# vmonardo/pnp-svrg

Hardware: AMD Instinct MI355X
Metric: PnP-SVRG inner-iters/sec, 256x256 CSMRI+DnCNN (higher is better)
Workload: dtype f32; 1 GPU; pnp_svrg (true SVRG direction, T2=10, mb=1000) on 256x256 CSMRI, 20% Bernoulli mask, DnCNN-17 prox (reference DnCNN_noise15 weights); batch_per_gpu=120, problems_total=120, parallelism=replicas x1 (no data-path collective)

## Files before the change

### pnp_svrg_amd/csrc/dncnn_wino44.hip

```cpp
#include "common.h"
#include "wino44.h"
#include "tilewalk.h"
#include <vector>
#include <utility>
#include <cstdlib>

namespace pnp {
namespace w44 {

using f32x4 = __attribute__((ext_vector_type(4))) float;
using f32x2 = __attribute__((ext_vector_type(2))) float;

constexpr int C = 64;
constexpr int TC = 64;
constexpr int PC = 72;
constexpr int KC = 8;
constexpr int NCH = C / KC;
template <int NG_> struct Geo {
    static constexpr int NG = NG_;
    static constexpr int TR = 4 * NG, PR = TR + 2;
    static constexpr int PLANE = NG == 2 ? 768 : 512;
    static constexpr int DBUF = KC * PLANE;
    static constexpr int PPW = DBUF / 256 / 4;
    static constexpr int VPL = 128 * NG;
    static constexpr int VBUF = 36 * VPL;
    static constexpr int LDS_FLOATS = 2 * DBUF + 2 * VBUF;
    static constexpr int NQ_AGPR = NG == 2 ? 64 : 36;
    static constexpr bool in_agpr(int g, int xi) { return g * 36 + xi < NQ_AGPR; }
};
constexpr int URING = 18;
constexpr unsigned DUMMY = 1u << 27;

__device__ __forceinline__ void bt6(float d0, float d1, float d2, float d3, float d4, float d5, float (&v)[6]) {
    const float t1 = __builtin_fmaf(-4.f, d2, d4), t2 = __builtin_fmaf(-4.f, d1, d3);
    const float t3 = d4 - d2, sd = d3 - d1;
    v[0] = __builtin_fmaf(4.f, d0, __builtin_fmaf(-5.f, d2, d4));
    v[1] = t1 + t2;
    v[2] = t1 - t2;
    v[3] = __builtin_fmaf(2.f, sd, t3);
    v[4] = __builtin_fmaf(-2.f, sd, t3);
    v[5] = __builtin_fmaf(4.f, d1, __builtin_fmaf(-5.f, d3, d5));
}
template <typename T> __device__ __forceinline__ void at6(T m0, T m1, T m2, T m3, T m4, T m5, T (&y)[4]) {
    const T s12 = m1 + m2, d12 = m1 - m2, s34 = m3 + m4, d34 = m3 - m4;
    y[0] = (m0 + s12) + s34;
    y[1] = 2.f * d34 + d12;
    y[2] = 4.f * s34 + s12;
    y[3] = (8.f * d34 + d12) + m5;
}

#define PNP_MFMA_PRE ""
#define PNP_MFMA_POST ""
template <bool AG> __device__ __forceinline__ void mfma(f32x4& acc, float w, float v) {
    if (AG) asm volatile(PNP_MFMA_PRE "v_mfma_f32_16x16x4_f32 %0, %1, %2, %0" PNP_MFMA_POST : "+a"(acc) : "v"(w), "v"(v));
    else asm volatile(PNP_MFMA_PRE "v_mfma_f32_16x16x4_f32 %0, %1, %2, %0" PNP_MFMA_POST : "+v"(acc) : "v"(w), "v"(v));
}
template <bool AG> __device__ __forceinline__ void mfma_first(f32x4& acc, float w, float v) {
    if (AG) asm volatile("v_mfma_f32_16x16x4_f32 %0, %1, %2, 0" PNP_MFMA_POST : "=&a"(acc) : "v"(w), "v"(v));
    else asm volatile("v_mfma_f32_16x16x4_f32 %0, %1, %2, 0" PNP_MFMA_POST : "=&v"(acc) : "v"(w), "v"(v));
}

typedef int i32x4 __attribute__((ext_vector_type(4)));
typedef __attribute__((address_space(3))) float lds_f;
typedef __attribute__((address_space(3))) f32x2 lds_f2;
typedef __attribute__((address_space(3))) f32x4 lds_f4;

__device__ __forceinline__ void dma_piece_asm(unsigned voff, i32x4 rsrc, unsigned lds_byte_addr) {
    asm volatile("s_mov_b32 m0, %2\n\ts_nop 0\n\tbuffer_load_dwordx4 %0, %1, 0 offen lds" :: "v"(voff), "s"(rsrc), "s"(lds_byte_addr) : "memory");
}

struct Patch {
    f32x2 a; f32x4 m; f32x2 e;
    f32x2 t[6][3];
    f32x2 v[6];
};
template <int NG_> struct Ctx {
    static constexpr int NG = NG_;
    using G = Geo<NG_>;
    f32x4 acc[NG_][36];
    f32x4 ur[URING];
    Patch P;
    f32x2 b[2][NG_];
    const lds_f* dsrc[2];
    lds_f* vdst[2];
    const lds_f* vsrc0[2];
    const lds_f* vsrc1[2];
    const __attribute__((address_space(1))) char* ucur;
    unsigned ulane;
    __device__ __forceinline__ f32x4 uload_next() {
        const f32x4 u = *(const __attribute__((address_space(1))) f32x4*)(ucur + ulane);
        ucur += 1024;
        asm volatile("" : "+s"(ucur));
        return u;
    }
};
#define PNP_SLOT() __builtin_amdgcn_sched_barrier(0)

template <int DPAR, int R, int HALF, typename CT> __device__ __forceinline__ void patch_load(CT& c) {
    const lds_f* row = c.dsrc[DPAR] + R * PC;
    if (HALF == 0) { c.P.a = *(const lds_f2*)(row + 2); c.P.e = *(const lds_f2*)(row + 8); }
    else c.P.m = *(const lds_f4*)(row + 4);
}
__device__ __forceinline__ f32x2 pk_sum_diff(f32x2 a) {
    f32x2 r;
    asm("v_pk_add_f32 %0, %1, %1 op_sel:[0,1] op_sel_hi:[1,0] neg_hi:[0,1]" : "=v"(r) : "v"(a));
    return r;
}
__device__ __forceinline__ f32x2 pk_hi_pm_2lo(f32x2 a) {
    f32x2 r;
    asm("v_pk_fma_f32 %0, %1, 2.0, %1 op_sel:[0,0,1] op_sel_hi:[0,0,1] neg_hi:[1,0,0]" : "=v"(r) : "v"(a));
    return r;
}
__device__ __forceinline__ void bt6_pk(f32x2 q0, f32x2 q1, f32x2 q2, f32x2 q3, f32x2 q4, f32x2 q5, f32x2 (&v)[6]) {
    const f32x2 t1 = q4 - 4.f * q2, t2 = q3 - 4.f * q1;
    const f32x2 t3 = q4 - q2, sd = q3 - q1;
    v[0] = 4.f * q0 + (q4 - 5.f * q2);
    v[1] = t1 + t2;
    v[2] = t1 - t2;
    v[3] = 2.f * sd + t3;
    v[4] = t3 - 2.f * sd;
    v[5] = 4.f * q1 + (q5 - 5.f * q3);
}
constexpr int col_pair(int sl) { return (sl - 6) / 2; }
constexpr bool is_col_slice(int sl) { return sl == 6 || sl == 8 || sl == 10; }
template <int SL, typename CT> __device__ __forceinline__ void slice_valu(CT& c) {
    Patch& P = c.P;
    if constexpr (SL < 6) {
        asm volatile("" :: "v"(P.a.x), "v"(P.e.y));
        const f32x2 p12 = {P.m.x, P.m.y}, p34 = {P.m.z, P.m.w};
        const f32x2 A = p34 - 4.f * p12;
        const f32x2 Bv = p34 - p12;
        P.t[SL][1] = pk_sum_diff(A);
        P.t[SL][2] = pk_hi_pm_2lo(Bv);
        float v0, v5;
        asm("v_fma_f32 %0, 4.0, %1, %2" : "=v"(v0) : "v"(P.a.y), "v"(__builtin_fmaf(-5.f, P.m.y, P.m.w)));
        asm("v_fma_f32 %0, 4.0, %1, %2" : "=v"(v5) : "v"(P.m.x), "v"(__builtin_fmaf(-5.f, P.m.z, P.e.x)));
        P.t[SL][0] = f32x2{v0, v5};
    } else if constexpr (is_col_slice(SL)) {
        constexpr int cp = col_pair(SL);
        bt6_pk(P.t[0][cp], P.t[1][cp], P.t[2][cp], P.t[3][cp], P.t[4][cp], P.t[5][cp], P.v);
    }
}
template <int DPAR, int SL, int N, typename CT> __device__ __forceinline__ void slice_lds(CT& c) {
    constexpr int VPL = CT::G::VPL;
    if constexpr (SL < 5) {
        if constexpr (N < 2) patch_load<DPAR, SL + 1, N>(c);
    } else if constexpr (is_col_slice(SL)) {
        constexpr int cp = col_pair(SL), xa = cp == 0 ? 0 : cp == 1 ? 1 : 3, xb = cp == 0 ? 5 : cp == 1 ? 2 : 4;
#pragma unroll
        for (int y = 2 * N; y < 2 * N + 2; ++y) {
            c.vdst[DPAR][(y * 6 + xa) * VPL] = c.P.v[y].x;
            c.vdst[DPAR][(y * 6 + xb) * VPL] = c.P.v[y].y;
        }
    }
}
template <int VPAR, int XI, int GR, typename CT> __device__ __forceinline__ void b_load(CT& c) {
    if constexpr (GR < CT::NG) {
        if (GR == 0) c.b[XI & 1][0] = *(const lds_f2*)(c.vsrc0[VPAR] + XI * CT::G::VPL);
        else c.b[XI & 1][GR] = *(const lds_f2*)(c.vsrc1[VPAR] + XI * CT::G::VPL);
    }
}
template <int K, int XI, int GR, typename CT> __device__ __forceinline__ void mfma_j0(CT& c, float u, f32x2 (&b)[CT::NG]) {
    if constexpr (GR < CT::NG) {
        if constexpr (K == 0) mfma_first<CT::G::in_agpr(GR, XI)>(c.acc[GR][XI], u, b[GR].x);
        else mfma<CT::G::in_agpr(GR, XI)>(c.acc[GR][XI], u, b[GR].x);
    }
}
template <int XI, int GR, typename CT> __device__ __forceinline__ void mfma_j1(CT& c, float u, f32x2 (&b)[CT::NG]) {
    if constexpr (GR < CT::NG) mfma<CT::G::in_agpr(GR, XI)>(c.acc[GR][XI], u, b[GR].y);
}

template <int K, int P, int VAR, typename CT, typename DMA> __device__ __forceinline__ void step(CT& c, DMA&& dma) {
    constexpr int X0 = 2 * P, X1 = 2 * P + 1, SQ = K * 18 + P;
    constexpr int VPAR = K & 1, DPAR = (K + 1) & 1, NG = CT::NG;
    const f32x4 u = c.ur[SQ % URING];
    f32x2 b0[NG], b1[NG];
#pragma unroll
    for (int g = 0; g < NG; ++g) b0[g] = c.b[0][g];
    mfma_j0<K, X0, 0>(c, u.x, b0);                   PNP_SLOT();
    if constexpr (VAR != 13 && VAR != 15) b_load<VPAR, X1, 0>(c);
    PNP_SLOT();
    mfma_j0<K, X0, 1>(c, u.x, b0);                   PNP_SLOT();
    if constexpr (VAR != 13 && VAR != 15) b_load<VPAR, X1, 1>(c);
    PNP_SLOT();
    mfma_j1<X0, 0>(c, u.y, b0);                      PNP_SLOT();
    if constexpr (VAR != 10 && VAR != 15) slice_valu<P>(c);
    PNP_SLOT();
    mfma_j1<X0, 1>(c, u.y, b0);                      PNP_SLOT();
    if constexpr (VAR != 14 && VAR != 15) slice_lds<DPAR, P, 0>(c);
    PNP_SLOT();
#pragma unroll
    for (int g = 0; g < NG; ++g) b1[g] = c.b[1][g];
    mfma_j0<K, X1, 0>(c, u.z, b1);                   PNP_SLOT();
    if constexpr (X1 + 1 < 36 && VAR != 13 && VAR != 15) b_load<VPAR, X1 + 1, 0>(c);
    PNP_SLOT();
    mfma_j0<K, X1, 1>(c, u.z, b1);                   PNP_SLOT();
    if constexpr (X1 + 1 < 36 && VAR != 13 && VAR != 15) b_load<VPAR, X1 + 1, 1>(c);
    PNP_SLOT();
    mfma_j1<X1, 0>(c, u.w, b1);                      PNP_SLOT();
    if constexpr (P < CT::G::PPW && VAR != 11 && VAR != 15) dma(P);
    if constexpr (VAR != 14 && VAR != 15) slice_lds<DPAR, P, 1>(c);
    PNP_SLOT();
    mfma_j1<X1, 1>(c, u.w, b1);                      PNP_SLOT();
    if constexpr (VAR != 14 && VAR != 15) slice_lds<DPAR, P, 2>(c);
    if constexpr (VAR != 12 && VAR != 15 && SQ + URING < NCH * 18) c.ur[SQ % URING] = c.uload_next();
    PNP_SLOT();
}
template <int K, int VAR, typename CT, typename DMA, int... P> __device__ __forceinline__ void chunk_steps(CT& c, DMA&& dma, std::integer_sequence<int, P...>) {
    (step<K, P, VAR>(c, dma), ...);
}
template <int K> constexpr int reloads_from(int p0) {
    int n = 0;
    for (int p = p0; p < 18; ++p) n += (K * 18 + p + URING < NCH * 18) ? 1 : 0;
    return n;
}
template <int K, bool STAMP, int VAR, typename CT, typename DMA> __device__ __forceinline__ void chunk(CT& c, DMA&& dma, unsigned long long& t_wait) {
    patch_load<(K + 1) & 1, 0, 0>(c);
    patch_load<(K + 1) & 1, 0, 1>(c);
    b_load<K & 1, 0, 0>(c);
    b_load<K & 1, 0, 1>(c);
    PNP_SLOT();
    chunk_steps<K, VAR>(c, dma, std::make_integer_sequence<int, 18>{});
    unsigned long long ta = 0;
    if (STAMP) ta = __builtin_amdgcn_s_memtime();
    asm volatile("s_waitcnt vmcnt(%0)" :: "n"(reloads_from<K>(CT::G::PPW)) : "memory");
    __syncthreads();
    if (STAMP) t_wait += __builtin_amdgcn_s_memtime() - ta;
}
template <bool STAMP, int VAR, typename CT, typename MK, int... K> __device__ __forceinline__ void all_chunks(CT& c, MK&& mk, unsigned long long& t_wait, std::integer_sequence<int, K...>) {
    (chunk<K, STAMP, VAR>(c, mk(std::integral_constant<int, K>{}), t_wait), ...);
}

template <int VPL> __device__ __forceinline__ void transform0(const float* dsrc, float* vdst) {
    float t[6][6];
#pragma unroll
    for (int r = 0; r < 6; ++r) {
        const float* row = dsrc + r * PC;
        bt6(row[3], row[4], row[5], row[6], row[7], row[8], t[r]);
    }
#pragma unroll
    for (int x = 0; x < 6; ++x) {
        float v[6];
        bt6(t[0][x], t[1][x], t[2][x], t[3][x], t[4][x], t[5][x], v);
#pragma unroll
        for (int y = 0; y < 6; ++y) vdst[(y * 6 + x) * VPL] = v[y];
    }
}

constexpr int FL_PATCH = 36;
constexpr int FL_BLK = 16 * FL_PATCH;
template <int NG, bool FL> constexpr int fl_lds_floats() { return FL ? C * 9 + NG * 4 * FL_BLK : 0; }

template <bool LEAKY, int NG = 2, bool STAMP = false, int VAR = 0, bool FL = false>
__global__ __launch_bounds__(256, 1) void k_mid_wino44(const float* __restrict__ in, float* __restrict__ out,
                                                       const float4* __restrict__ upack, const float* __restrict__ bias,
                                                       int H, int W, int ntiles, float slope,
                                                       unsigned long long* __restrict__ stamps = nullptr, int tile0 = 0,
                                                       const float* __restrict__ wlast = nullptr, float* __restrict__ part = nullptr) {
    using G = Geo<NG>;
    constexpr int TR = G::TR, PR = G::PR, PLANE = G::PLANE, DBUF = G::DBUF, PPW = G::PPW, VPL = G::VPL, VBUF = G::VBUF;
    static_assert(!(FL && LEAKY), "the fused last layer is built for the ReLU net");
    __shared__ __attribute__((aligned(16))) float lds[G::LDS_FLOATS + fl_lds_floats<NG, FL>()];
    const int tid = threadIdx.x, lane = tid & 63, wv = __builtin_amdgcn_readfirstlane(tid >> 6);
    const int tiles_x = W / TC, units_per_img = tiles_x * (H / 8);
    auto region = [&](int u, int& b, int& ty0, int& tx0) {
        const int t = tile0 + (NG == 2 ? u : u >> 1);
        b = t / units_per_img;
        const int t2 = t - b * units_per_img;
        ty0 = (t2 / tiles_x) * 8 + (NG == 2 ? 0 : 4 * (u & 1));
        tx0 = (t2 % tiles_x) * TC;
    };

    float bv[4];
#pragma unroll
    for (int r = 0; r < 4; ++r) bv[r] = bias[16 * wv + 4 * (lane >> 4) + r];

    const int tc = lane & 15, j = (lane >> 4) & 1, g = NG == 2 ? lane >> 5 : 0;
    const int d_off = 4 * ((2 * wv + j) * (PLANE / 4) + g * PC + tc);
    const ptrdiff_t hw4 = (ptrdiff_t)4 * H * W, w4 = (ptrdiff_t)4 * W;
    const unsigned st_off = 4u * (unsigned)(4 * (lane >> 4) * H * W + 4 * tc);
    const int v_off = g * 128 + wv * 32 + tc * 2 + j;

    unsigned pdesc[PPW];
#pragma unroll
    for (int i = 0; i < PPW; ++i) {
        const int q = (wv + 4 * i) * 64 + lane;
        const int c = q / (PLANE / 4), r = q - c * (PLANE / 4);
        const int ry = r / 18, cx4 = 4 * (r - ry * 18);
        const unsigned edge = (ry == 0 ? 1u : 0u) | (ry == PR - 1 ? 2u : 0u) | (cx4 == 0 ? 4u : 0u) | (cx4 == TC + 4 ? 8u : 0u);
        pdesc[i] = r < PR * 18 ? ((unsigned)((c * H + ry) * W + cx4) | (edge << 28)) : DUMMY;
    }
    const unsigned lds0 = (unsigned)(size_t)(__attribute__((address_space(3))) float*)lds;
    struct TileDma { size_t base; unsigned voff[PPW]; };
    const size_t chunk_bytes = (size_t)KC * H * W * 4;
    auto tile_dma = [&](int t) {
        TileDma td;
        int b, ty0, tx0;
        region(t, b, ty0, tx0);
        td.base = (size_t)in + 4 * ((((size_t)b * C) * H + ty0 - 1) * (size_t)W + tx0 - 4);
        const unsigned bad = t < ntiles ? ((((ty0 == 0 ? 1u : 0u) | (ty0 + TR == H ? 2u : 0u) | (tx0 == 0 ? 4u : 0u) | (tx0 + TC == W ? 8u : 0u)) << 28) | DUMMY)
                                        : 0xFFFFFFFFu;
#pragma unroll
        for (int i = 0; i < PPW; ++i) td.voff[i] = (pdesc[i] & bad) == 0u ? 4u * (pdesc[i] & 0x07FFFFFFu) : 0x80000000u;
        return td;
    };
    auto chunk_rsrc = [&](const TileDma& td, int k) {
        const size_t base = td.base + (size_t)k * chunk_bytes;
        i32x4 rs;
        rs.x = (int)(unsigned)base; rs.y = (int)(unsigned)(base >> 32) & 0xFFFF; rs.z = (int)0x80000000u; rs.w = 0x00020000;
        return rs;
    };
    auto dma_piece = [&](const TileDma& td, i32x4 rs, int buf, int i) {
        dma_piece_asm(td.voff[i], rs, lds0 + 4u * (unsigned)(buf * DBUF + (wv + 4 * i) * 256));
    };

    float* const dbuf = lds;
    float* const vbuf = lds + 2 * DBUF;

    Ctx<NG> c;
    lds_f* const ldsp = (lds_f*)lds;
    c.dsrc[0] = ldsp + d_off;                     c.dsrc[1] = ldsp + DBUF + d_off;
    c.vdst[0] = ldsp + 2 * DBUF + v_off;          c.vdst[1] = ldsp + 2 * DBUF + VBUF + v_off;
    c.vsrc0[0] = ldsp + 2 * DBUF + 2 * lane;      c.vsrc0[1] = ldsp + 2 * DBUF + VBUF + 2 * lane;
    c.vsrc1[0] = c.vsrc0[0] + 128;                c.vsrc1[1] = c.vsrc0[1] + 128;
    asm volatile("" : "+v"(c.vsrc1[0]), "+v"(c.vsrc1[1]));
    const __attribute__((address_space(1))) char* const ubase = (const __attribute__((address_space(1))) char*)upack + (size_t)(wv * NCH * 18) * 1024;
    c.ucur = ubase;
    c.ulane = 16u * lane;

    const TileWalk tw_ = tile_walk(ntiles);
    int tile = tw_.first;
    const int limit = tw_.limit < ntiles ? tw_.limit : ntiles;
    float* const flw = lds + G::LDS_FLOATS;
    float* const flx = flw + C * 9;
    if constexpr (FL)
        for (int i = tid; i < C * 9; i += 256) flw[i] = wlast[i];
    {
        const TileDma td0 = tile_dma(tile < limit ? tile : ntiles);
#pragma unroll
        for (int i = 0; i < PPW; ++i) dma_piece(td0, chunk_rsrc(td0, 0), 0, i);
#pragma unroll
        for (int i = 0; i < PPW; ++i) dma_piece(td0, chunk_rsrc(td0, 1), 1, i);
#pragma unroll
        for (int i = 0; i < URING; ++i) c.ur[i] = c.uload_next();
        asm volatile("s_waitcnt vmcnt(0)" ::: "memory");
        __syncthreads();
        transform0<VPL>(dbuf + d_off, vbuf + v_off);
        __syncthreads();
    }

    unsigned long long t0 = 0, r0 = 0, t_wait = 0, t_epi = 0;
    if (STAMP) { t0 = __builtin_amdgcn_s_memtime(); r0 = __builtin_amdgcn_s_memrealtime(); }
    for (; tile < limit; tile += tw_.step) {
        asm volatile("" : "+v"(c.ulane));
        int b, ty0, tx0;
        region(tile, b, ty0, tx0);
        const int ntile = tile + tw_.step < limit ? tile + tw_.step : ntiles;

        const TileDma cur = tile_dma(tile), nxt = tile_dma(ntile);
        all_chunks<STAMP, VAR>(c, [&](auto kc) {
            constexpr int K = decltype(kc)::value;
            const TileDma& td = K + 2 < NCH ? cur : nxt;
            const i32x4 rs = chunk_rsrc(td, (K + 2) % NCH);
            return [&, rs](int piece) { dma_piece(td, rs, K & 1, piece); };
        }, t_wait, std::make_integer_sequence<int, NCH>{});

        unsigned long long te = 0;
        if (STAMP) te = __builtin_amdgcn_s_memtime();
        asm volatile("; W44_EPILOGUE_BEGIN\n\ts_nop 15\n\ts_nop 7" ::: "memory");
#pragma unroll
        for (int g2 = 0; g2 < NG; ++g2)
#pragma unroll
            for (int xi = 0; xi < 36; xi += 4) {
                if (G::in_agpr(g2, xi)) asm volatile("" : "+a"(c.acc[g2][xi]), "+a"(c.acc[g2][xi + 1]), "+a"(c.acc[g2][xi + 2]), "+a"(c.acc[g2][xi + 3]));
                else asm volatile("" : "+v"(c.acc[g2][xi]), "+v"(c.acc[g2][xi + 1]), "+v"(c.acc[g2][xi + 2]), "+v"(c.acc[g2][xi + 3]));
            }
        unsigned so = st_off;
        asm volatile("" : "+v"(so));
        __attribute__((address_space(1))) char* const ob = (__attribute__((address_space(1))) char*)out + 4 * ((((size_t)b * C + 16 * wv) * H + ty0) * (size_t)W + tx0);
        float q[FL_PATCH];
#pragma unroll
        for (int blk = 0; blk < 2 * NG; ++blk) {
            {
                const int g2 = NG == 2 ? 1 - (blk >> 1) : 0, pi = blk & 1;
                float wr[2][9];
                if constexpr (FL) {
                    if (pi == 0)
#pragma unroll
                        for (int i = 0; i < FL_PATCH; ++i) q[i] = 0.f;
                    const float* wc = flw + (16 * wv + 4 * (lane >> 4) + 2 * pi) * 9;
#pragma unroll
                    for (int t = 0; t < 9; ++t) { wr[0][t] = wc[t]; wr[1][t] = wc[9 + t]; }
                }
                if (blk == 2 * NG - 1) {
                    c.ucur = ubase;
#pragma unroll
                    for (int i = 0; i < URING; ++i) c.ur[i] = c.uload_next();
                    __builtin_amdgcn_sched_barrier(0);
                }
                const f32x2 bias2 = {bv[2 * pi], bv[2 * pi + 1]};
                __attribute__((address_space(1))) char* oc = ob + (ptrdiff_t)(2 * pi) * hw4 + (ptrdiff_t)(4 * g2) * w4;
                asm volatile("" : "+s"(oc));
                f32x2 s[6][4];
#pragma unroll
                for (int x = 0; x < 6; ++x) {
                    f32x2 m[6];
#pragma unroll
                    for (int y = 0; y < 6; ++y) {
                        const f32x4 q = c.acc[g2][6 * y + x];
                        m[y] = pi ? f32x2{q.z, q.w} : f32x2{q.x, q.y};
                    }
                    if (x == 1) m[1] += bias2;
                    at6(m[0], m[1], m[2], m[3], m[4], m[5], s[x]);
                    if (x & 1) __builtin_amdgcn_sched_barrier(0);
                }
#pragma unroll
                for (int r = 0; r < 4; ++r) {
                    f32x2 y[4];
                    at6(s[0][r], s[1][r], s[2][r], s[3][r], s[4][r], s[5][r], y);
                    f32x4 v0, v1;
                    if (LEAKY) {
                        v0.x = fmaxf(y[0].x, slope * y[0].x); v0.y = fmaxf(y[1].x, slope * y[1].x);
                        v0.z = fmaxf(y[2].x, slope * y[2].x); v0.w = fmaxf(y[3].x, slope * y[3].x);
                        v1.x = fmaxf(y[0].y, slope * y[0].y); v1.y = fmaxf(y[1].y, slope * y[1].y);
                        v1.z = fmaxf(y[2].y, slope * y[2].y); v1.w = fmaxf(y[3].y, slope * y[3].y);
                    } else {
                        v0.x = fmaxf(y[0].x, 0.f); v0.y = fmaxf(y[1].x, 0.f); v0.z = fmaxf(y[2].x, 0.f); v0.w = fmaxf(y[3].x, 0.f);
                        v1.x = fmaxf(y[0].y, 0.f); v1.y = fmaxf(y[1].y, 0.f); v1.z = fmaxf(y[2].y, 0.f); v1.w = fmaxf(y[3].y, 0.f);
                    }
                    if constexpr (FL) {
                        const float a0[4] = {v0.x, v0.y, v0.z, v0.w}, a1[4] = {v1.x, v1.y, v1.z, v1.w};
#pragma unroll
                        for (int dy = 0; dy < 3; ++dy)
#pragma unroll
                            for (int dx = 0; dx < 3; ++dx)
#pragma unroll
                                for (int k = 0; k < 4; ++k) {
                                    float& d = q[(r + 2 - dy) * 6 + k + 2 - dx];
                                    d = __builtin_fmaf(wr[0][dy * 3 + dx], a0[k], d);
                                    d = __builtin_fmaf(wr[1][dy * 3 + dx], a1[k], d);
                                }
                    } else {
                        *(__attribute__((address_space(1))) f32x4*)(oc + so) = v0;
                        oc += hw4;
                        asm volatile("" : "+s"(oc));
                        *(__attribute__((address_space(1))) f32x4*)(oc + so) = v1;
                        oc += w4 - hw4;
                        asm volatile("" : "+s"(oc));
                    }
                    if (r & 1) __builtin_amdgcn_sched_barrier(0);
                }
                if constexpr (FL) {
                    if (pi == 1) {
                        const bool h32 = (lane & 32) != 0, h16 = (lane & 16) != 0;
                        float k1[18], k2[9];
#pragma unroll
                        for (int i = 0; i < 18; ++i) {
                            const float mine = h32 ? q[18 + i] : q[i], give = h32 ? q[i] : q[18 + i];
                            k1[i] = mine + __shfl_xor(give, 32);
                        }
#pragma unroll
                        for (int i = 0; i < 9; ++i) {
                            const float mine = h16 ? k1[9 + i] : k1[i], give = h16 ? k1[i] : k1[9 + i];
                            k2[i] = mine + __shfl_xor(give, 16);
                        }
                        float* const xd = flx + (g2 * 4 + wv) * FL_BLK + tc * FL_PATCH + 9 * (lane >> 4);
#pragma unroll
                        for (int i = 0; i < 9; ++i) xd[i] = k2[i];
                    }
                }
            }
        }
        if constexpr (FL) {
            __syncthreads();
            float* const pb = part + (((size_t)b * (H / 4) + ty0 / 4) * (size_t)(W / 4) + tx0 / 4) * FL_PATCH;
            for (int e = tid; e < NG * FL_BLK; e += 256) {
                const int g2 = e >= FL_BLK ? 1 : 0, rem = e - g2 * FL_BLK;
                const float* xs = flx + g2 * 4 * FL_BLK + rem;
                pb[(size_t)g2 * (W / 4) * FL_PATCH + rem] = ((xs[0] + xs[FL_BLK]) + xs[2 * FL_BLK]) + xs[3 * FL_BLK];
            }
        }
        asm volatile("; W44_EPILOGUE_END" ::: "memory");
        if (STAMP) t_epi += __builtin_amdgcn_s_memtime() - te;
    }
    if (STAMP && tid == 0) {
        stamps[4 * blockIdx.x] = __builtin_amdgcn_s_memtime() - t0;
        stamps[4 * blockIdx.x + 1] = __builtin_amdgcn_s_memrealtime() - r0;
        stamps[4 * blockIdx.x + 2] = t_wait;
        stamps[4 * blockIdx.x + 3] = t_epi;
    }
}

}

bool wino44_supports(int H, int W) { return H % 8 == 0 && W % w44::TC == 0; }

size_t wino44_layer_bytes() { return (size_t)4 * w44::NCH * 18 * 64 * 4 * sizeof(float); }

void wino44_pack(const float* w_mid, int n_mid, void* out_) {
    static const double G[6][3] = {{1.0 / 4, 0, 0}, {-1.0 / 6, -1.0 / 6, -1.0 / 6}, {-1.0 / 6, 1.0 / 6, -1.0 / 6},
                                   {1.0 / 24, 1.0 / 12, 1.0 / 6}, {1.0 / 24, -1.0 / 12, 1.0 / 6}, {0, 0, 1}};
    float* out = (float*)out_;
    for (int l = 0; l < n_mid; ++l)
        for (int wv = 0; wv < 4; ++wv)
            for (int k = 0; k < w44::NCH; ++k)
                for (int lane = 0; lane < 64; ++lane)
                    for (int j = 0; j < 2; ++j) {
                        const int cout = 16 * wv + (lane & 15), cin = w44::KC * k + 2 * (lane >> 4) + j;
                        const float* g = w_mid + (((size_t)l * w44::C + cout) * w44::C + cin) * 9;
                        for (int xy = 0; xy < 6; ++xy)
                            for (int xx = 0; xx < 6; ++xx) {
                                double u = 0;
                                for (int dy = 0; dy < 3; ++dy)
                                    for (int dx = 0; dx < 3; ++dx) u += G[xy][dy] * G[xx][dx] * (double)g[dy * 3 + dx];
                                const int xi = 6 * xy + xx, p = xi >> 1, e = 2 * (xi & 1) + j;
                                out[((((size_t)(l * 4 + wv) * w44::NCH + k) * 18 + p) * 64 + lane) * 4 + e] = (float)u;
                            }
                    }
}

int wino44_layer(const ConvLayerArgs& a) {
    PNP_CHECK_ARG(a.part == nullptr || (a.slope == 0.f && a.wlast != nullptr), "the fused last layer needs ReLU and w_last");
    const float *in = a.in, *bias = a.bias, *wlast = a.wlast;
    float *out = a.out, *part = a.part;
    const int H = a.H, W = a.W, num_cu = a.num_cu, force = a.force_rows, batch = a.batch;
    const float slope = a.slope;
    const hipStream_t s = a.s;
    const int units = batch * (H / 8) * (W / w44::TC);
    int full = force == 1 ? 0 : force == 2 ? units : (units / num_cu) * num_cu;
    if (force == 0 && 2 * (units - full) > num_cu) full = units;
    const float4* up = (const float4*)(a.w44_override ? a.w44_override : (const float*)a.w + a.layer * wino44_layer_bytes() / sizeof(float));
    if (full > 0) {
        const int grid = full < num_cu ? full : num_cu;
        if (part) w44::k_mid_wino44<false, 2, false, 0, true><<<grid, 256, 0, s>>>(in, out, up, bias, H, W, full, 0.f, nullptr, 0, wlast, part);
        else if (slope != 0.f) w44::k_mid_wino44<true, 2><<<grid, 256, 0, s>>>(in, out, up, bias, H, W, full, slope, nullptr, 0);
        else w44::k_mid_wino44<false, 2><<<grid, 256, 0, s>>>(in, out, up, bias, H, W, full, 0.f, nullptr, 0);
        PNP_CHECK_LAUNCH();
    }
    if (full < units) {
        const int n1 = 2 * (units - full), grid = n1 < num_cu ? n1 : num_cu;
        if (part) w44::k_mid_wino44<false, 1, false, 0, true><<<grid, 256, 0, s>>>(in, out, up, bias, H, W, n1, 0.f, nullptr, full, wlast, part);
        else if (slope != 0.f) w44::k_mid_wino44<true, 1><<<grid, 256, 0, s>>>(in, out, up, bias, H, W, n1, slope, nullptr, full);
        else w44::k_mid_wino44<false, 1><<<grid, 256, 0, s>>>(in, out, up, bias, H, W, n1, 0.f, nullptr, full);
        PNP_CHECK_LAUNCH();
    }
    return PNP_OK;
}

int wino44_debug_clock(const ConvLayerArgs& a, int reps, std::vector<double>& cycles, std::vector<double>& ticks) {
    const int ntiles = a.batch * (a.H / 8) * (a.W / w44::TC);
    const int grid = ntiles < a.num_cu ? ntiles : a.num_cu;
    const float *in = a.in, *bias = a.bias;
    float* out = a.out;
    const int H = a.H, W = a.W;
    const hipStream_t s = a.s;
    const float* upack_layer = (const float*)a.w + a.layer * wino44_layer_bytes() / sizeof(float);
    std::vector<unsigned long long> h;
    const int rc = read_stamps(s, grid, 4, [&](unsigned long long* stamps_dev) {
        for (int i = 0; i < reps - 1; ++i)
            w44::k_mid_wino44<false, 2><<<grid, 256, 0, s>>>(in, out, (const float4*)upack_layer, bias, H, W, ntiles, 0.f);
        const int var = getenv("PNP_W44_VAR") ? atoi(getenv("PNP_W44_VAR")) : 0;
        if (var == 0) w44::k_mid_wino44<false, 2, true><<<grid, 256, 0, s>>>(in, out, (const float4*)upack_layer, bias, H, W, ntiles, 0.f, stamps_dev);
#ifdef PNP_W44_ABLATIONS
#define PNP_W44_ABL(V) else if (var == V) w44::k_mid_wino44<false, 2, true, V><<<grid, 256, 0, s>>>(in, out, (const float4*)upack_layer, bias, H, W, ntiles, 0.f, stamps_dev);
        PNP_W44_ABL(10) PNP_W44_ABL(11) PNP_W44_ABL(12) PNP_W44_ABL(13) PNP_W44_ABL(14) PNP_W44_ABL(15)
#undef PNP_W44_ABL
#endif
        else PNP_CHECK_ARG(false, "PNP_W44_VAR: this library was built without -DPNP_W44_ABLATIONS");
        PNP_CHECK_LAUNCH();
        return PNP_OK;
    }, h, cycles, ticks);
    if (rc != PNP_OK) return rc;
    if (getenv("PNP_DEBUG_STAMPS")) {
        double wsum = 0, esum = 0, rsum = 0;
        for (int i = 0; i < grid; ++i) { wsum += (double)(h[4 * i + 2] & 0xFFFFFFFFull); rsum += (double)(h[4 * i + 2] >> 32); esum += h[4 * i + 3]; }
        fprintf(stderr, "[k_mid_wino44 stamps] mean cycles per WG: chunk-end wait + barrier %.0f  epilogue %.0f  (mode 6: steps 0..5 of the chunks %.0f)\n",
                wsum / grid, esum / grid, rsum / grid);
    }
    return PNP_OK;
}

}
```

Before: 5251 inner-iters/s.

## Interleave V-tile layout for two block rows and reschedule NG=2 step pipeline

For the two-block-row (NG=2) Winograd kernel, the V buffer layout is interleaved so both groups' B operands come from one 128-bit LDS read instead of two 64-bit reads. A dedicated step2 schedule redistributes patch loads, DMA pieces, VALU transforms and V writes across the MFMA slots so that each interleaved slot holds at most one LDS or DMA operation. The vmcnt wait count is adjusted to match the shifted U reload points. This is meant to reduce LDS instruction count and smooth issue between the matrix and vector pipes, but it adds a more intricate schedule that is correct only for PPW=6.

```diff
diff --git a/pnp_svrg_amd/csrc/dncnn_wino44.hip b/pnp_svrg_amd/csrc/dncnn_wino44.hip
--- a/pnp_svrg_amd/csrc/dncnn_wino44.hip
+++ b/pnp_svrg_amd/csrc/dncnn_wino44.hip
@@ -84,7 +84,6 @@
     const lds_f* dsrc[2];
     lds_f* vdst[2];
     const lds_f* vsrc0[2];
-    const lds_f* vsrc1[2];
     const __attribute__((address_space(1))) char* ucur;
     unsigned ulane;
     __device__ __forceinline__ f32x4 uload_next() {
@@ -141,23 +140,26 @@
         bt6_pk(P.t[0][cp], P.t[1][cp], P.t[2][cp], P.t[3][cp], P.t[4][cp], P.t[5][cp], P.v);
     }
 }
+template <int DPAR, int SL, int Y, typename CT> __device__ __forceinline__ void v_write(CT& c) {
+    constexpr int VPL = CT::G::VPL;
+    constexpr int cp = col_pair(SL), xa = cp == 0 ? 0 : cp == 1 ? 1 : 3, xb = cp == 0 ? 5 : cp == 1 ? 2 : 4;
+    c.vdst[DPAR][(Y * 6 + xa) * VPL] = c.P.v[Y].x;
+    c.vdst[DPAR][(Y * 6 + xb) * VPL] = c.P.v[Y].y;
+}
 template <int DPAR, int SL, int N, typename CT> __device__ __forceinline__ void slice_lds(CT& c) {
-    constexpr int VPL = CT::G::VPL;
     if constexpr (SL < 5) {
         if constexpr (N < 2) patch_load<DPAR, SL + 1, N>(c);
     } else if constexpr (is_col_slice(SL)) {
-        constexpr int cp = col_pair(SL), xa = cp == 0 ? 0 : cp == 1 ? 1 : 3, xb = cp == 0 ? 5 : cp == 1 ? 2 : 4;
-#pragma unroll
-        for (int y = 2 * N; y < 2 * N + 2; ++y) {
-            c.vdst[DPAR][(y * 6 + xa) * VPL] = c.P.v[y].x;
-            c.vdst[DPAR][(y * 6 + xb) * VPL] = c.P.v[y].y;
-        }
-    }
-}
-template <int VPAR, int XI, int GR, typename CT> __device__ __forceinline__ void b_load(CT& c) {
-    if constexpr (GR < CT::NG) {
-        if (GR == 0) c.b[XI & 1][0] = *(const lds_f2*)(c.vsrc0[VPAR] + XI * CT::G::VPL);
-        else c.b[XI & 1][GR] = *(const lds_f2*)(c.vsrc1[VPAR] + XI * CT::G::VPL);
+        v_write<DPAR, SL, 2 * N>(c);
+        v_write<DPAR, SL, 2 * N + 1>(c);
+    }
+}
+template <int VPAR, int XI, typename CT> __device__ __forceinline__ void b_load(CT& c) {
+    if constexpr (CT::NG == 1) c.b[XI & 1][0] = *(const lds_f2*)(c.vsrc0[VPAR] + XI * CT::G::VPL);
+    else {
+        const f32x4 q = *(const lds_f4*)(c.vsrc0[VPAR] + XI * CT::G::VPL);
+        c.b[XI & 1][0] = f32x2{q.x, q.y};
+        c.b[XI & 1][CT::NG - 1] = f32x2{q.z, q.w};
     }
 }
 template <int K, int XI, int GR, typename CT> __device__ __forceinline__ void mfma_j0(CT& c, float u, f32x2 (&b)[CT::NG]) {
@@ -171,59 +173,102 @@
 }
 
 template <int K, int P, int VAR, typename CT, typename DMA> __device__ __forceinline__ void step(CT& c, DMA&& dma) {
+    static_assert(CT::NG == 1, "two block rows: step2");
     constexpr int X0 = 2 * P, X1 = 2 * P + 1, SQ = K * 18 + P;
-    constexpr int VPAR = K & 1, DPAR = (K + 1) & 1, NG = CT::NG;
+    constexpr int VPAR = K & 1, DPAR = (K + 1) & 1;
     const f32x4 u = c.ur[SQ % URING];
-    f32x2 b0[NG], b1[NG];
-#pragma unroll
-    for (int g = 0; g < NG; ++g) b0[g] = c.b[0][g];
+    f32x2 b0[1] = {c.b[0][0]}, b1[1];
     mfma_j0<K, X0, 0>(c, u.x, b0);                   PNP_SLOT();
-    if constexpr (VAR != 13 && VAR != 15) b_load<VPAR, X1, 0>(c);
-    PNP_SLOT();
-    mfma_j0<K, X0, 1>(c, u.x, b0);                   PNP_SLOT();
-    if constexpr (VAR != 13 && VAR != 15) b_load<VPAR, X1, 1>(c);
+    if constexpr (VAR != 13 && VAR != 15) b_load<VPAR, X1>(c);
     PNP_SLOT();
     mfma_j1<X0, 0>(c, u.y, b0);                      PNP_SLOT();
     if constexpr (VAR != 10 && VAR != 15) slice_valu<P>(c);
     PNP_SLOT();
-    mfma_j1<X0, 1>(c, u.y, b0);                      PNP_SLOT();
     if constexpr (VAR != 14 && VAR != 15) slice_lds<DPAR, P, 0>(c);
     PNP_SLOT();
-#pragma unroll
-    for (int g = 0; g < NG; ++g) b1[g] = c.b[1][g];
+    b1[0] = c.b[1][0];
     mfma_j0<K, X1, 0>(c, u.z, b1);                   PNP_SLOT();
-    if constexpr (X1 + 1 < 36 && VAR != 13 && VAR != 15) b_load<VPAR, X1 + 1, 0>(c);
-    PNP_SLOT();
-    mfma_j0<K, X1, 1>(c, u.z, b1);                   PNP_SLOT();
-    if constexpr (X1 + 1 < 36 && VAR != 13 && VAR != 15) b_load<VPAR, X1 + 1, 1>(c);
+    if constexpr (X1 + 1 < 36 && VAR != 13 && VAR != 15) b_load<VPAR, X1 + 1>(c);
     PNP_SLOT();
     mfma_j1<X1, 0>(c, u.w, b1);                      PNP_SLOT();
     if constexpr (P < CT::G::PPW && VAR != 11 && VAR != 15) dma(P);
     if constexpr (VAR != 14 && VAR != 15) slice_lds<DPAR, P, 1>(c);
     PNP_SLOT();
-    mfma_j1<X1, 1>(c, u.w, b1);                      PNP_SLOT();
     if constexpr (VAR != 14 && VAR != 15) slice_lds<DPAR, P, 2>(c);
     if constexpr (VAR != 12 && VAR != 15 && SQ + URING < NCH * 18) c.ur[SQ % URING] = c.uload_next();
     PNP_SLOT();
 }
+template <int DPAR, int P, int S, int VAR, typename CT, typename DMA> __device__ __forceinline__ void slot2(CT& c, DMA&& dma) {
+    constexpr bool LDS = VAR != 14 && VAR != 15, DM = VAR != 11 && VAR != 15;
+    if constexpr (P == 0) {
+        if constexpr (S < 2 && LDS) patch_load<DPAR, 0, S>(c);
+        if constexpr (S == 3 && DM) dma(0);
+    } else if constexpr (P < 6) {
+        if constexpr (S == 0 && DM) dma(P);
+        if constexpr ((S == 1 || S == 2) && LDS) patch_load<DPAR, P, S - 1>(c);
+    } else if constexpr (P >= 7 && P <= 12 && LDS) {
+        constexpr int SL = 6 + 2 * ((P - 7) / 2), Y = (P & 1) ? S - 1 : S + 3;
+        if constexpr (Y >= 0 && Y < 6) v_write<DPAR, SL, Y>(c);
+    }
+}
+template <int P, typename CT> __device__ __forceinline__ void valu2(CT& c) {
+    if constexpr (P >= 1 && P <= 6) slice_valu<P - 1>(c);
+    else if constexpr (P == 7 || P == 9 || P == 11) slice_valu<P - 1>(c);
+}
+template <int K, int P, int VAR, typename CT, typename DMA> __device__ __forceinline__ void step2(CT& c, DMA&& dma) {
+    static_assert(CT::NG == 2 && CT::G::PPW == 6, "one DMA piece in each of the steps 0..5");
+    constexpr int X0 = 2 * P, X1 = 2 * P + 1, SQ = K * 18 + P;
+    constexpr int VPAR = K & 1, DPAR = (K + 1) & 1;
+    const f32x4 u = c.ur[SQ % URING];
+    f32x2 b0[2] = {c.b[0][0], c.b[0][1]}, b1[2];
+    mfma_j0<K, X0, 0>(c, u.x, b0);                   PNP_SLOT();
+    if constexpr (VAR != 13 && VAR != 15) b_load<VPAR, X1>(c);
+    PNP_SLOT();
+    mfma_j0<K, X0, 1>(c, u.x, b0);                   PNP_SLOT();
+    slot2<DPAR, P, 0, VAR>(c, dma);
+    PNP_SLOT();
+    mfma_j1<X0, 0>(c, u.y, b0);                      PNP_SLOT();
+    if constexpr (VAR != 10 && VAR != 15) valu2<P>(c);
+    if constexpr (P == 0 && K > 0 && VAR != 12 && VAR != 15 && SQ - 1 + URING < NCH * 18) c.ur[(SQ - 1) % URING] = c.uload_next();
+    PNP_SLOT();
+    mfma_j1<X0, 1>(c, u.y, b0);                      PNP_SLOT();
+    slot2<DPAR, P, 1, VAR>(c, dma);
+    PNP_SLOT();
+    b1[0] = c.b[1][0]; b1[1] = c.b[1][1];
+    mfma_j0<K, X1, 0>(c, u.z, b1);                   PNP_SLOT();
+    if constexpr (X1 + 1 < 36 && VAR != 13 && VAR != 15) b_load<VPAR, X1 + 1>(c);
+    PNP_SLOT();
+    mfma_j0<K, X1, 1>(c, u.z, b1);                   PNP_SLOT();
+    slot2<DPAR, P, 2, VAR>(c, dma);
+    PNP_SLOT();
+    mfma_j1<X1, 0>(c, u.w, b1);                      PNP_SLOT();
+    slot2<DPAR, P, 3, VAR>(c, dma);
+    PNP_SLOT();
+    mfma_j1<X1, 1>(c, u.w, b1);                      PNP_SLOT();
+    if constexpr (P < 17 && VAR != 12 && VAR != 15 && SQ + URING < NCH * 18) c.ur[SQ % URING] = c.uload_next();
+    PNP_SLOT();
+}
 template <int K, int VAR, typename CT, typename DMA, int... P> __device__ __forceinline__ void chunk_steps(CT& c, DMA&& dma, std::integer_sequence<int, P...>) {
-    (step<K, P, VAR>(c, dma), ...);
-}
-template <int K> constexpr int reloads_from(int p0) {
+    if constexpr (CT::NG == 2) (step2<K, P, VAR>(c, dma), ...);
+    else (step<K, P, VAR>(c, dma), ...);
+}
+template <int K> constexpr int reloads_of(int p0, int p1) {
     int n = 0;
-    for (int p = p0; p < 18; ++p) n += (K * 18 + p + URING < NCH * 18) ? 1 : 0;
+    for (int p = p0; p <= p1; ++p) n += (K * 18 + p + URING < NCH * 18) ? 1 : 0;
     return n;
 }
 template <int K, bool STAMP, int VAR, typename CT, typename DMA> __device__ __forceinline__ void chunk(CT& c, DMA&& dma, unsigned long long& t_wait) {
-    patch_load<(K + 1) & 1, 0, 0>(c);
-    patch_load<(K + 1) & 1, 0, 1>(c);
-    b_load<K & 1, 0, 0>(c);
-    b_load<K & 1, 0, 1>(c);
+    if constexpr (CT::NG == 1) {
+        patch_load<(K + 1) & 1, 0, 0>(c);
+        patch_load<(K + 1) & 1, 0, 1>(c);
+    }
+    b_load<K & 1, 0>(c);
     PNP_SLOT();
     chunk_steps<K, VAR>(c, dma, std::make_integer_sequence<int, 18>{});
     unsigned long long ta = 0;
     if (STAMP) ta = __builtin_amdgcn_s_memtime();
-    asm volatile("s_waitcnt vmcnt(%0)" :: "n"(reloads_from<K>(CT::G::PPW)) : "memory");
+    constexpr int PPW = CT::G::PPW, younger = CT::NG == 2 ? reloads_of<K>(PPW - 1, 16) : reloads_of<K>(PPW, 17);
+    asm volatile("s_waitcnt vmcnt(%0)" :: "n"(younger) : "memory");
     __syncthreads();
     if (STAMP) t_wait += __builtin_amdgcn_s_memtime() - ta;
 }
@@ -279,7 +324,7 @@
     const int d_off = 4 * ((2 * wv + j) * (PLANE / 4) + g * PC + tc);
     const ptrdiff_t hw4 = (ptrdiff_t)4 * H * W, w4 = (ptrdiff_t)4 * W;
     const unsigned st_off = 4u * (unsigned)(4 * (lane >> 4) * H * W + 4 * tc);
-    const int v_off = g * 128 + wv * 32 + tc * 2 + j;
+    const int v_off = NG == 2 ? wv * 64 + tc * 4 + g * 2 + j : wv * 32 + tc * 2 + j;
 
     unsigned pdesc[PPW];
 #pragma unroll
@@ -321,9 +366,8 @@
     lds_f* const ldsp = (lds_f*)lds;
     c.dsrc[0] = ldsp + d_off;                     c.dsrc[1] = ldsp + DBUF + d_off;
     c.vdst[0] = ldsp + 2 * DBUF + v_off;          c.vdst[1] = ldsp + 2 * DBUF + VBUF + v_off;
-    c.vsrc0[0] = ldsp + 2 * DBUF + 2 * lane;      c.vsrc0[1] = ldsp + 2 * DBUF + VBUF + 2 * lane;
-    c.vsrc1[0] = c.vsrc0[0] + 128;                c.vsrc1[1] = c.vsrc0[1] + 128;
-    asm volatile("" : "+v"(c.vsrc1[0]), "+v"(c.vsrc1[1]));
+    asm volatile("" : "+v"(c.vdst[0]), "+v"(c.vdst[1]));
+    c.vsrc0[0] = ldsp + 2 * DBUF + 2 * NG * lane; c.vsrc0[1] = ldsp + 2 * DBUF + VBUF + 2 * NG * lane;
     const __attribute__((address_space(1))) char* const ubase = (const __attribute__((address_space(1))) char*)upack + (size_t)(wv * NCH * 18) * 1024;
     c.ucur = ubase;
     c.ulane = 16u * lane;
```

Result: faster. 5330 inner-iters/s (median of 6 runs) (+1.5%).
